# abignoli/EdgeGraph3D

Hardware: AMD Instinct MI355X
Metric: triangulated edge-points/sec (higher is better)
Workload: dtype f64

## Files before the change

edgegraph3d_amd/build.py:

```python
import os
import subprocess
import sys

ROOT = os.path.dirname(os.path.dirname(os.path.abspath(__file__)))
PKG = os.path.join(ROOT, "edgegraph3d_amd")
HOST_DIR = os.path.join(PKG, "host")
CSRC_DIR = os.path.join(PKG, "csrc")
INC_DIR = os.path.join(ROOT, "include")

HOST_LIB = os.path.join(PKG, "libeg3d_host.so")
HIP_LIB = os.path.join(PKG, "libeg3d.so")

HOST_FLAGS = ["-O2", "-std=c++17", "-fPIC", "-shared", "-ffp-contract=off", "-fno-fast-math", "-fopenmp", "-Wall"]
HIP_OPT_FLAGS = ["-O2", "-fno-slp-vectorize", "-fno-vectorize", "-mllvm", "-disable-machine-licm", "-mllvm", "-disable-lsr",
                 "-mllvm", "-enable-pre=false", "-mllvm", "-enable-load-pre=false", "-mllvm", "-enable-misched=false"]
HIP_FLAGS = ["--offload-arch=gfx950"] + HIP_OPT_FLAGS + ["-std=c++17", "-fPIC", "-shared", "-ffp-contract=off",
             "-fno-fast-math", "-fhip-fp32-correctly-rounded-divide-sqrt", "-fno-gpu-rdc",
             "-Wall", "-Wno-unused-function", "-Wno-unused-variable", "-Wno-unused-but-set-variable"]


def _newer(target, sources):
    if not os.path.exists(target):
        return True
    t = os.path.getmtime(target)
# ... 111 lines not shown
    src = os.path.join(PKG, "rccl", "eg3d_rccl.hip")
    deps = [src] + _all_sources(INC_DIR, (".h",)) + _all_sources(os.path.join(PKG, "rccl"), (".h",))
    if force or _newer(RCCL_LIB, deps):
        hipcc = os.environ.get("HIPCC", "/opt/rocm/bin/hipcc")
        _run([hipcc, "--offload-arch=gfx950", "-O2", "-std=c++17", "-fPIC", "-shared", "-I", INC_DIR, src,
              "-L/opt/rocm/lib", "-lrccl", "-Wl,-rpath,/opt/rocm/lib", "-o", RCCL_LIB])
    return RCCL_LIB


RESOURCE_BOUNDS = {
    "k3b_expand_t<4, 0, 0>": {"vgpr_spill_count": 120, "private_segment_fixed_size": 224, "group_segment_fixed_size": 10240},
    "k3b_expand_t<4, 0, 1>": {"vgpr_spill_count": 360, "private_segment_fixed_size": 400, "group_segment_fixed_size": 10240},
    "k3b_expand_t<4, 1, 2>": {"vgpr_spill_count": 140, "private_segment_fixed_size": 256, "group_segment_fixed_size": 10240},
    "k3a_orient": {"vgpr_spill_count": 0, "group_segment_fixed_size": 12800},
    "k3a_follow_spec": {"vgpr_spill_count": 0, "group_segment_fixed_size": 12800},
    "k5_gn_filter": {"vgpr_spill_count": 0},
    "k5_gn_filter<unsigned int, true>": {"vgpr_spill_count": 0, "private_segment_fixed_size": 0, "vgpr_count": 57,
                                         "group_segment_fixed_size": 47124},
    "k5_gn_filter<unsigned long, false>": {"vgpr_spill_count": 0, "private_segment_fixed_size": 0, "group_segment_fixed_size": 48164},
    "k6_compact_scatter": {"vgpr_spill_count": 0, "private_segment_fixed_size": 0, "group_segment_fixed_size": 3104},
    "k7_dedup_claim": {"vgpr_spill_count": 0, "private_segment_fixed_size": 0, "group_segment_fixed_size": 2048},
    "k7_dedup_keep": {"vgpr_spill_count": 0, "private_segment_fixed_size": 0, "group_segment_fixed_size": 16},
    "k8_": {"vgpr_spill_count": 0, "private_segment_fixed_size": 0, "group_segment_fixed_size": 0},
    "k9_": {"vgpr_spill_count": 0, "sgpr_spill_count": 0, "private_segment_fixed_size": 0, "group_segment_fixed_size": 2048},
    "k10_": {"vgpr_spill_count": 0, "sgpr_spill_count": 0, "private_segment_fixed_size": 0, "group_segment_fixed_size": 2048},
    "k11_": {"vgpr_spill_count": 0, "sgpr_spill_count": 0, "private_segment_fixed_size": 0, "group_segment_fixed_size": 32},
    "k12_": {"sgpr_spill_count": 0, "private_segment_fixed_size": 0, "group_segment_fixed_size": 0},
    "k12_keys": {"vgpr_spill_count": 0}, "k12_heads": {"vgpr_spill_count": 0}, "k12_compact": {"vgpr_spill_count": 0},
    "k12_view_off": {"vgpr_spill_count": 0}, "k12_common": {"vgpr_spill_count": 0}, "k12_samples": {"vgpr_spill_count": 0},
    "k12_select": {"vgpr_spill_count": 0}, "k12_final": {"vgpr_spill_count": 0},
# ... 103 lines not shown
```

edgegraph3d_amd/csrc/eg3d_api.hip:

```cpp
#include <hip/hip_runtime.h>
#include <hipcub/hipcub.hpp>

#include <algorithm>
#include <cstdio>
#include <cstdlib>

#include <atomic>
#include <chrono>
#include <cmath>
#include <cstring>
#include <memory>
#include <mutex>
#include <string>
#include <thread>
#include <vector>

#include "../../include/eg3d_host.h"
#include "eg3d_api_internal.h"
#include "eg3d_host_copy.h"

thread_local std::string eg3d::api::g_err;
extern "C" const char* eg3d_last_error(void) { return g_err.c_str(); }

static std::atomic<int64_t> g_live_device_bytes{0};
// ... 931 lines not shown

extern "C" int eg3d_probe_sections_raw(eg3d_ctx* c, double* sum16, uint32_t* n_chains) {
  if (!c || !sum16) return EG3D_ERR_ARG;
  std::vector<ChainOut> co(c->last_nc ? c->last_nc : 1);
  if (c->last_nc) HIP_TRY(hipMemcpy(co.data(), c->b_couts.p, sizeof(ChainOut) * c->last_nc, hipMemcpyDeviceToHost));
  for (int k = 0; k < 16; k++) sum16[k] = 0;
  for (uint32_t j = 0; j < c->last_nc; j++)
    for (int k = 0; k < 16; k++) sum16[k] += (double)co[j].tsec[k];
  if (n_chains) *n_chains = c->last_nc;
  return EG3D_OK;
}

#ifndef EG3D_ONE_SECTION
namespace eg3d { int gn_dbg_read(unsigned long long* out, int reset); }
extern "C" int eg3d_probe_gn(unsigned long long* out128, int reset) { return eg3d::gn_dbg_read(out128, reset); }
#endif

extern "C" int eg3d_probe_hyp_sections(eg3d_ctx* c, double* sum, double* slowest, uint32_t* counts) {
  if (!c || !sum || !slowest || !counts) return EG3D_ERR_ARG;
  const uint32_t n = c->last_nhyp;
  std::vector<HypResult> r(n ? n : 1);
  if (n) HIP_TRY(hipMemcpy(r.data(), c->b_res.p, sizeof(HypResult) * n, hipMemcpyDeviceToHost));
  for (int k = 0; k < 6; k++) sum[k] = slowest[k] = 0;
  for (int k = 0; k < 5; k++) counts[k] = 0;
  counts[0] = n;
  for (uint32_t h = 0; h < n; h++) {
    if (r[h].status & HYP_TRI) counts[1]++;
    if (r[h].status & HYP_D1) counts[2]++;
    if (r[h].status & HYP_D2) counts[3]++;
    if (hyp_compatible(r[h].status, r[h].n1, r[h].n2)) counts[4]++;
// ... 15 lines not shown
```

edgegraph3d_amd/csrc/eg3d_api_internal.h:

```cpp
#pragma once
#include <hip/hip_runtime.h>

#include <algorithm>
#include <chrono>
#include <cstdlib>
#include <cstring>
#include <initializer_list>
#include <memory>
#include <mutex>
#include <string>
#include <vector>

#include "../../include/eg3d.h"
#include "eg3d_kernels.h"
#include "eg3d_k8_replay.h"
#include "eg3d_k9_polymatch.h"
#include "eg3d_k10_simgraph.h"
#include "eg3d_k11_louvain.h"

#define EG3D_API_BEGIN namespace eg3d { namespace api __attribute__((visibility("hidden"))) {
#define EG3D_API_END }}

EG3D_API_BEGIN
extern thread_local std::string g_err;
// ... 175 lines not shown
  WorkBuf prim_tmp;
  WorkBuf k8_cnt, k8_slot, k8_last, k8_firstof, k8_flag, k8_rank, k8_lastof, k8_plid, k8_key[2], k8_val[2], k8_map, k8_sflag, k8_pos;
  WorkBuf g_nodeX, g_nodept, g_pls, g_ple, g_conoff, g_conpl, g_ivoff, g_ivss, g_ivsxy, g_ives, g_ivexy;
  WorkBuf k9_svseed, k9_cnt, k9_pl, k9_dist, k9_acc, k9_accoff, k9_first, k9_parent, k9_root, k9_ckey, k9_rank, k9_key[2], k9_ctr,
      k9_ref, k9_rowoff, k9_plids;
  WorkBuf k10_svseed, k10_cnt, k10_off, k10_pair[2], k10_crkey, k10_cpoff, k10_cpview, k10_cppl, k10_croff, k10_crpoint, k10_weight, k10_vis,
      k10_npairs, k10_pairoff, k10_nkey[2], k10_nodeof, k10_nodeg, k10_nodeview, k10_nodepl, k10_edge[2], k10_dkey[2], k10_dval[2],
      k10_adjoff, k10_adjnode, k10_ctr;
  WorkBuf k11[K11B_COUNT];
  uint32_t louvain_log2_slots = 0;
  uint64_t simgraph_pair_budget = 0;
  int replay_table_bits = 0;
  uint32_t n_pl = 0, n_vtx = 0;
  WorkBuf b_sets_off, b_sets_ids;
  WorkBuf b_fscratch, b_queue, b_items;
  WorkBuf b_pools, b_stage_pts, b_stage_obs, b_stage_used;
  uint32_t slots_per_xcd = 0;
  int k3c_per_cu = 0;
  bool k3b_long_latched = false;
  uint32_t max_pl_vtx = 0;
  uint64_t stage_cap_pts = 0, stage_cap_obs = 0;
  double hits_per_list = 4.0;
  bool hits_learned = false;
  hipEvent_t ea[8], eb[8];
  hipEvent_t ecopy[7] = {nullptr, nullptr, nullptr, nullptr, nullptr, nullptr, nullptr};
  uint32_t chain_cap = 384, pool_cap = 0, hyp_cap = 160;
  uint32_t n_simd = 0;
  int wall_clock_khz = 0;
  double arena_per_hyp = 16.0;
  void* pinned = nullptr;
// ... 112 lines not shown
```

edgegraph3d_amd/csrc/eg3d_api_match.hip:

```cpp
#include <sys/mman.h>

#include <atomic>
#include <condition_variable>
#include <cstdio>
#include <shared_mutex>
#include <thread>

#include "eg3d_api_internal.h"
#include "eg3d_host_copy.h"

#ifndef EG3D_D2H_CHUNK
#define EG3D_D2H_CHUNK ((size_t)16 << 20)
#endif
#define EG3D_D2H_CHUNK_SMALL ((size_t)2 << 20)
#define EG3D_D2H_BIG_CLOUD ((size_t)96 << 20)
#ifndef EG3D_D2H_RING
#define EG3D_D2H_RING 4
#endif
static int ensure_d2h_ring(eg3d_ctx* c, size_t cloud_bytes) {
  const size_t want = cloud_bytes >= EG3D_D2H_BIG_CLOUD ? EG3D_D2H_CHUNK : EG3D_D2H_CHUNK_SMALL;
  if (c->pinned && c->ring_chunk >= want) return EG3D_OK;
  if (c->pinned) (void)hipHostFree(c->pinned);
  c->pinned = nullptr;
  c->ring_chunk = c->pinned_cap = 0;
// ... 303 lines not shown

int follow_and_select(eg3d_ctx* c, BatchState& B, HostOut& H) {
  hipStream_t st = c->stream;
  const uint32_t nt = B.n_tasks;
  BUF_TRY(c->b_res.ensure(sizeof(HypResult) * (B.n_hyp + 1)));
  const uint32_t eng_waves_max = c->n_simd * (uint32_t)(c->tune.k3a_engine_waves > 0 ? c->tune.k3a_engine_waves : 2);
  uint32_t eng_lanes = 64;
  if (c->tune.k3a_engine_lanes > 0)
    eng_lanes = (uint32_t)std::min(64, c->tune.k3a_engine_lanes);
  else
    while (eng_lanes > 8 && (uint64_t)eng_waves_max * (eng_lanes / 2) >= B.n_hyp) eng_lanes /= 2;
  const uint32_t eng_waves = std::max<uint32_t>(1, std::min<uint32_t>(eng_waves_max, (B.n_hyp + eng_lanes - 1) / eng_lanes));
  BUF_TRY(c->b_fscratch.ensure(sizeof(HPoint) * std::min<uint32_t>(c->hyp_cap, EG3D_K3A_STAGE_POINTS) * ((size_t)eng_waves * 64)));
  BUF_TRY(c->b_queue.ensure(4 * sizeof(uint32_t)));
  BUF_TRY(c->b_items.ensure(sizeof(uint32_t) * 2 * ((size_t)B.n_hyp + 1)));
  uint32_t arena_cap = std::max<uint32_t>(1u << 16, std::min<uint64_t>((uint64_t)((double)B.n_hyp * c->arena_per_hyp) + 1, 1ull << 26));
  if (c->tune.arena_cap0) arena_cap = c->tune.arena_cap0;
  Counters hc;
  BUF_TRY(c->b_cs_task.ensure(sizeof(ChainSeed) * (nt + 1)));
  BUF_TRY(c->b_valid.ensure(sizeof(uint32_t) * (nt + 1)));
  BUF_TRY(c->b_chain_off.ensure(sizeof(uint32_t) * (nt + 1)));
  for (int attempt = 0;; attempt++) {
    BUF_TRY(c->b_arena.ensure(sizeof(HPoint) * (size_t)arena_cap));
    HIP_TRY(hipMemsetAsync(c->b_ctr.p, 0, 2 * sizeof(uint32_t), st));
    HIP_TRY(hipEventRecord(c->ea[3], st));
    HIP_TRY(hipMemsetAsync(c->b_queue.p, 0, 4 * sizeof(uint32_t), st));
    launch_k3a_engine(st, eng_waves, eng_waves, eng_lanes, c->ds, B.a, c->b_tasks.as<TaskDesc>(), c->b_hyp_off.as<uint32_t>(),
                      B.n_hyp, c->b_res.as<HypResult>(), c->b_fscratch.as<HPoint>(), c->hyp_cap, c->b_arena.as<HPoint>(),
                      arena_cap, c->b_ctr.as<Counters>(), c->b_queue.as<uint32_t>(), c->b_items.as<uint32_t>());
    HIP_TRY(hipEventRecord(c->eb[3], st));
    HIP_TRY(hipMemsetAsync(c->b_valid.as<uint32_t>() + nt, 0, sizeof(uint32_t), st));
    HIP_TRY(hipEventRecord(c->ea[4], st));
    launch_k3s(st, nt, c->b_hyp_off.as<uint32_t>(), c->b_res.as<HypResult>(), c->b_cs_task.as<ChainSeed>(),
               c->b_valid.as<uint32_t>());
    BUF_TRY(scan_queue_u32(c, c->b_valid.as<uint32_t>(), c->b_chain_off.as<uint32_t>(), nt + 1, 0));
    Readback rb(c);
    const int ic = rb.add(c->b_ctr.p, sizeof(Counters) / 4);
    const int it = rb.add(c->b_chain_off.as<uint32_t>() + nt, 1);
    const int iw = rb.add(c->b_scanchk.as<uint32_t>(), 1);
    rb.clear_after(c->b_scanchk.as<uint32_t>());
    BUF_TRY(rb.run());
    memcpy(&hc, rb.item(ic), sizeof(Counters));
    if (c->tune.trace_arena)
// ... 1003 lines not shown
```

edgegraph3d_amd/csrc/eg3d_k3a_engine.h:

```cpp
#pragma once
#include "eg3d_dev_pipeline.h"

#include "eg3d_dev_coopgn.h"

namespace eg3d {

#ifdef EG3D_GN_COUNTERS
#define K3A_T0() unsigned long long kt_[3] = {0, 0, 0}, kc_[4] = {0, 0, 0, 0}, kt0_ = __builtin_readcyclecounter(), kt1_
#define K3A_T(i) (kt1_ = __builtin_readcyclecounter(), kt_[i] += kt1_ - kt0_, kt0_ = kt1_)
#define K3A_C(i, v) (kc_[i] += (v))
#define K3A_TEND(kern)                                                \
  if (lane == 0) {                                                    \
    for (int q_ = 0; q_ < 3; q_++) EG3D_GN_DBG(113 + 7 * (kern) + q_, kt_[q_]); \
    for (int q_ = 0; q_ < 4; q_++) EG3D_GN_DBG(116 + 7 * (kern) + q_, kc_[q_]); \
  }
#else
#define K3A_T0() ((void)0)
#define K3A_T(i) ((void)0)
#define K3A_C(i, v) ((void)0)
#define K3A_TEND(kern) ((void)0)
#endif

#define EG3D_K3A_STAGE EG3D_K3A_STAGE_POINTS
#ifndef EG3D_K3A_SPEC
#define EG3D_K3A_SPEC 32
#endif

struct K3aShared {
  Obs req[64][3];
  float resX[64][3];
  uint32_t resF[64];
// ... 36 lines not shown
  }
};

__device__ __forceinline__ uint32_t k3a_slots_per_lane(uint32_t n_working) {
  uint32_t k = 64u / n_working, p = 1;
  while (p * 2 <= k && p * 2 <= (uint32_t)EG3D_K3A_SPEC) p *= 2;
  return p;
}

__device__ __forceinline__ void k3a_serve(K3aShared& sh, const DevScene& s, uint32_t lane) {
  __syncthreads();
  if (sh.reqM[lane] & 1u) {
    const Obs o[3] = {sh.req[lane][0], sh.req[lane][1], sh.req[lane][2]};
    float X[3] = {0.0f, 0.0f, 0.0f};
    uint32_t f = 0;
    const bool ok = triangulate3(s.cam_P, o, X, f);
    sh.resX[lane][0] = X[0];
    sh.resX[lane][1] = X[1];
    sh.resX[lane][2] = X[2];
    sh.resF[lane] = (ok ? 1u : 0u) | (f << 8);
  }
  __syncthreads();
}

__device__ __forceinline__ HPoint k3a_point_of_slot(const K3aShared& sh, uint32_t slot) {
  HPoint hp;
  hp.X[0] = sh.resX[slot][0];
  hp.X[1] = sh.resX[slot][1];
  hp.X[2] = sh.resX[slot][2];
  hp.nobs = 3;
  hp.o[0] = sh.req[slot][0];
  hp.o[1] = sh.req[slot][1];
  hp.o[2] = sh.req[slot][2];
  hp.pad = 0;
  return hp;
}

enum : uint32_t { K3A_IDLE = 0, K3A_GEN = 1, K3A_REQ = 2, K3A_END = 3 };
enum : uint32_t { K3A_TRI0 = 0, K3A_ORIENT = 1, K3A_REPLAY = 2, K3A_OPP = 3 };

__global__ void __launch_bounds__(64, EG3D_K3A_WAVES) k3a_orient(DevScene s, StageAView a, const TaskDesc* tasks,
                                                                 const uint32_t* hyp_off, uint32_t n_hyp, HypResult* res,
                                                                 uint32_t cap, HPoint* arena, uint32_t arena_cap,
                                                                 Counters* ctr, uint32_t* queue, uint32_t lanes_per_wave,
                                                                 uint32_t* items, uint32_t* n_items) {
  __shared__ K3aShared sh;
  const uint32_t lane = threadIdx.x;
  const K3aLane L{&sh, lane};
  const unsigned long long lt = (1ull << lane) - 1ull;
  uint32_t st = K3A_IDLE, phase = K3A_TRI0;
  bool exhausted = lane >= lanes_per_wave;
  uint32_t h = 0, t_cur = 0, e = 0, rounds = 0, alive = 0, reqmask = 0, okmask = 0, flags = 0, status = 0;
  uint32_t n1 = 0, n2 = 0, i_rep = 0, base = 0xffffffffu;
  uint32_t dead_round = 0xffffffffu;
  bool arena_ok = false;
  int32_t view[3] = {0, 0, 0};
  uint32_t pl[3] = {0, 0, 0};
  uint32_t dirA = 0, dirB[2] = {0, 0}, dirC[2] = {0, 0};
  uint32_t d1[3] = {0, 0, 0}, d2[3] = {0, 0, 0};
  float X0[3] = {0.0f, 0.0f, 0.0f};
  auto to_hits = [&](const Obs c[3]) {
    PlPt p;
    p.seg = c[0].seg;
    p.x = c[0].x;
    p.y = c[0].y;
// ... 25 lines not shown
    sh.req[slot][0] = o;
    o.view = (uint32_t)view[1];
    o.pl = pl[1];
    o.seg = pB.seg;
    o.x = pB.x;
    o.y = pB.y;
    sh.req[slot][1] = o;
    o.view = (uint32_t)view[2];
    o.pl = pl[2];
    o.seg = pC.seg;
    o.x = pC.x;
    o.y = pC.y;
    sh.req[slot][2] = o;
    sh.reqM[slot] = 1u | ((uint32_t)q << 8) | (round_off << 10);
  };
  K3A_T0();

  for (;;) {
    const unsigned long long working = __ballot(!(st == K3A_IDLE && exhausted));
    if (!working) break;
    K3A_C(0, 1);
    K3A_C(2, __popcll(working));
    const uint32_t K = k3a_slots_per_lane((uint32_t)__popcll(working));
    const uint32_t slot0 = (uint32_t)__popcll(working & lt) * K;
    sh.reqM[lane] = 0;
    __syncthreads();
    uint32_t n_issued = 0;
    if (st == K3A_END) {
      bool finish = false, to_d1 = false, restart = false;
      if (phase == K3A_TRI0) {
        if (okmask & 1u) {
          status |= HYP_TRI;
          e = 0;
          phase = K3A_ORIENT;
          restart = true;
        } else {
          finish = true;
        }
      } else if (phase == K3A_ORIENT) {
        const int amount = __popc(alive);
        if (amount > 1) {
          st = K3A_GEN;
        } else if (amount == 1) {
          to_d1 = true;
        } else if (e == 0) {
          e = 1;
          reload_hits();
          restart = true;
        } else {
          finish = true;
        }
      } else if (phase == K3A_REPLAY) {
        if (i_rep < n1) {
          st = K3A_GEN;
        } else if (e == 0) {
          phase = K3A_OPP;
          dirA = d2[0];
          dirB[0] = d2[1];
          dirC[0] = d2[2];
          alive = 1u;
          reload_hits();
          st = K3A_GEN;
        } else {
          finish = true;
        }
      } else {
        finish = true;
      }
      if (restart) {
        rounds = 0;
        alive = 15u;
        dirA = sh.plr[0][e == 0 ? 2 : 3][lane];
        dirB[0] = sh.plr[1][2][lane];
        dirB[1] = sh.plr[1][3][lane];
        dirC[0] = sh.plr[2][2][lane];
        dirC[1] = sh.plr[2][3][lane];
        st = K3A_GEN;
      }
      if (to_d1) {
        const int qs = __ffs((int)alive) - 1;
        const PlRef pa = L.polyline(s, 0), pb = L.polyline(s, 1), pc = L.polyline(s, 2);
        status |= HYP_D1;
        d1[0] = dirA;
        d1[1] = dirB[qs >> 1];
        d1[2] = dirC[qs & 1];
        d2[0] = (pa.start == d1[0]) ? pa.end : pa.start;
        d2[1] = (pb.start == d1[1]) ? pb.end : pb.start;
        d2[2] = (pc.start == d1[2]) ? pc.end : pc.start;
        if (rounds > cap) flags |= 4u;
        n1 = rounds < cap ? rounds : cap;
        const uint32_t need = n1 + (e == 0 ? 1u : 0u);
        base = atomicAdd(&ctr->arena_used, need);
        arena_ok = base + need <= arena_cap;
        if (!arena_ok) atomicOr(&ctr->flags, CTR_ARENA_OVERFLOW);
        phase = K3A_REPLAY;
        i_rep = 0;
        dirA = d1[0];
        dirB[0] = d1[1];
        dirC[0] = d1[2];
        alive = 1u;
        reload_hits();
        st = K3A_GEN;
      }
      if (finish) {
        HypResult r;
        r.status = status;
        r.n1 = n1;
        r.n2 = n2;
        for (int k = 0; k < 3; k++) {
          r.dirs1[k] = d1[k];
          r.dirs2[k] = d2[k];
          r.X[k] = X0[k];
        }
        r.flags = flags;
        r.pts1_off = ((status & HYP_D1) && arena_ok) ? base : 0xffffffffu;
        r.pts2_off = ((status & HYP_D2) && arena_ok) ? base + n1 : 0xffffffffu;
        res[h] = r;
        if (flags) atomicOr(&ctr->flags, flags);
        if ((status & HYP_D1) && arena_ok) {
          const uint32_t cnt = (status & HYP_D2) ? 2u : 1u;
          const uint32_t at = atomicAdd(n_items, cnt);
          items[at] = 2u * h;
          if (cnt == 2u) items[at + 1] = 2u * h + 1u;
        }
        st = K3A_IDLE;
      }
    }
    if (st == K3A_IDLE && !exhausted) {
      const uint32_t i = atomicAdd(queue, 1u);
      if (i >= n_hyp) {
        exhausted = true;
      } else {
        h = i;
        t_cur = find_owner(hyp_off, a.n_tasks, h);
        const TaskDesc d = tasks[t_cur];
        Obs c[3];
        hypothesis_hits(a, d, t_cur, h - hyp_off[t_cur], c);
        for (int k = 0; k < 3; k++) {
          view[k] = (int32_t)c[k].view;
          pl[k] = c[k].pl;
          L.load_polyline(s, k, view[k], pl[k]);
        }
        to_hits(c);
        status = 0;
        flags = 0;
        n1 = n2 = 0;
        base = 0xffffffffu;
        arena_ok = false;
        for (int k = 0; k < 3; k++) d1[k] = d2[k] = 0;
        X0[0] = X0[1] = X0[2] = 0.0f;
        phase = K3A_TRI0;
        reqmask = 1u;
        okmask = 0;
        st = K3A_REQ;
      }
    }
    dead_round = 0xffffffffu;
    if (st == K3A_GEN) {
      uint32_t walkers = alive;
      for (uint32_t round_off = 0;; round_off++) {
        uint32_t fl = 0, m = walkers;
        const PlRef pa = L.polyline(s, 0);
        PlPt q;
        const uint32_t w = walk_by_distance_pf(pa, L.get(0), dirA, EG3D_FOLLOW_STEP, q);
        if (w & WALK_BAD_DIR) fl |= 8u;
        if (w & WALK_EXTREME) {
          m = 0;
        } else {
          L.set(0, q);
// ... 10 lines not shown
              }
              pk = L.polyline(s, k);
            }
            if (!(m & users)) continue;
            PlPt r;
            const uint32_t wr = walk_by_line_pf(pk, L.get(2 * k - 1 + j), k == 1 ? dirB[j] : dirC[j], la, lb, lc, false, 0.0f,
                                                0.0f, r);
            if (wr & WALK_BAD_DIR) fl |= 8u;
            if (wr & WALK_FOUND)
              L.set(2 * k - 1 + j, r);
            else
              m &= ~users;
          }
        }
        if (phase != K3A_REPLAY) flags |= fl;
        if (round_off == 0) {
          reqmask = m;
          okmask = 0;
          if (!m) {
            if (phase == K3A_REPLAY) n1 = i_rep;
            if (phase == K3A_ORIENT) {
              alive = 0;
              rounds++;
            }
            st = K3A_END;
            break;
          }
          st = K3A_REQ;
          while (reqmask && n_issued < K) {
            const int qq = __ffs((int)reqmask) - 1;
// ... 54 lines not shown
        for (uint32_t j = 0; j < n_issued && !decided; j++) {
          const uint32_t mq = sh.reqM[slot0 + j], f = sh.resF[slot0 + j];
          const uint32_t q = (mq >> 8) & 3u, ro = mq >> 10;
          if (ro != cur) {
            alive = cur == 0 ? okmask : (alive & okmask);
            okmask = 0;
            rounds++;
            cur = ro;
            if (__popc(alive) <= 1) {
              decided = true;
              break;
            }
          }
          if (cur != 0 && !((alive >> q) & 1u)) continue;
          flags |= f >> 8;
          if (f & 1u) okmask |= 1u << q;
        }
        if (decided) {
          st = K3A_END;
        } else if (reqmask) {
          st = K3A_REQ;
        } else {
          alive = cur == 0 ? okmask : (alive & okmask);
          okmask = 0;
          rounds++;
          if (__popc(alive) > 1 && dead_round != 0xffffffffu) {
            alive = 0;
            rounds++;
          }
          st = K3A_END;
        }
      } else {
        const uint32_t f = sh.resF[slot0];
        flags |= f >> 8;
        if (f & 1u) {
          okmask |= 1u;
          if (phase == K3A_TRI0) {
            X0[0] = sh.resX[slot0][0];
            X0[1] = sh.resX[slot0][1];
            X0[2] = sh.resX[slot0][2];
          } else {
            status |= HYP_D2;
            n2 = 1;
            if (arena_ok) arena[base + n1] = k3a_point_of_slot(sh, slot0);
          }
        }
        st = K3A_END;
      }
    }
    K3A_T(2);
  }
  K3A_TEND(0);
}

template <class T>
__device__ __forceinline__ T k3a_pick(const T a[3], int i) {
  return i == 0 ? a[0] : i == 1 ? a[1] : a[2];
}
__device__ __forceinline__ bool k3a_follow_request(const DevScene& s, const K3aLane& L, const int32_t view3[3],
                                                   int st_start, const uint32_t dirs[3], const int32_t ids[3],
// ... 138 lines not shown
        }
        sh.reqM[slot] = 1u | ((uint32_t)st_used << 8) | (fl << 16);
        n_req++;
        for (int k = 0; k < 3; k++) {
          bview[k] = nview[k];
          bpl[k] = npl[k];
          L.set(3 + k, sel_pt[k]);
        }
        st0 = 0;
      }
    }
    K3A_T(0);
    K3A_C(0, 1);
    K3A_C(2, __popcll(working));
    K3A_C(1, __popcll(__ballot(sh.reqM[lane] & 1u)));
    k3a_serve(sh, s, lane);
    K3A_T(1);
    if (have) {
      bool finish = false;
      uint32_t j = 0;
      for (; j < n_req; j++) {
        const uint32_t slot = slot0 + j;
        const uint32_t m = sh.reqM[slot], f = sh.resF[slot];
        flags |= (m >> 16) | (f >> 8);
        if (f & 1u) {
          if (n_init + n_new >= cap) {
            flags |= 4u;
            finish = true;
            break;
          }
// ... 78 lines not shown
```

edgegraph3d_amd/csrc/eg3d_kernels.h:

```cpp
#pragma once
#include <hip/hip_runtime.h>
#include <stdint.h>

#include "eg3d_dev_pipeline.h"

namespace eg3d {

struct SeedsDev {
  const uint32_t* trk_off;
  const int32_t* trk_view;
  const float* trk_xy;
};

__device__ __forceinline__ void seed_obs_in_view(const SeedsDev& sd, uint32_t t0, uint32_t k, int32_t view, float& x,
                                                 float& y) {
  x = 0.f;
  y = 0.f;
  for (uint32_t i = 0; i < k; i++)
    if (sd.trk_view[t0 + i] == view) {
      x = sd.trk_xy[2 * (t0 + i)];
      y = sd.trk_xy[2 * (t0 + i) + 1];
    }
}

// ... 34 lines not shown
               Obs* hits, uint32_t hits_cap, uint32_t stage_cap, Counters* ctr);
struct SetsDev {
  uint32_t n_views;
  const uint32_t* row_off;
  const uint32_t* pl_ids;
};
void launch_n1_samples(hipStream_t st, bool fill, DevScene s, SetsDev sets, uint32_t n_rows, uint32_t item_begin,
                       uint32_t n_items, uint32_t* sample_cnt, const uint32_t* sample_off, Obs* samples,
                       uint32_t* task_seed, uint32_t* task_entry, uint32_t* task_hit, uint32_t* task_list_off,
                       uint32_t* task_row0, Counters* ctr);
void launch_n1_hits(hipStream_t st, bool fill, DevScene s, SetsDev sets, uint32_t n_tasks, const Obs* samples,
                    const uint32_t* task_row0, uint32_t* list_cnt, const uint32_t* list_ptr, Obs* hits, Counters* ctr);
void launch_task_setup(hipStream_t st, StageAView a, const int32_t* map_view, const uint32_t* map_entry,
                       const uint32_t* map_n, TaskDesc* tasks, uint32_t* n_hyp);
#define EG3D_K3A_STAGE_POINTS 16u
void launch_k3a_engine(hipStream_t st, uint32_t orient_waves, uint32_t follow_waves, uint32_t lanes_per_wave, DevScene s,
                       StageAView a, const TaskDesc* tasks, const uint32_t* hyp_off, uint32_t n_hyp, HypResult* res,
                       HPoint* follow_scratch, uint32_t hyp_cap, HPoint* arena, uint32_t arena_cap, Counters* ctr,
                       uint32_t* queue3, uint32_t* items);
void launch_k3s(hipStream_t st, uint32_t n_tasks, const uint32_t* hyp_off, const HypResult* res, ChainSeed* per_task,
                uint32_t* valid);
void launch_compact_chains(hipStream_t st, uint32_t n_tasks, const ChainSeed* per_task, const uint32_t* valid,
                           const uint32_t* chain_off, ChainSeed* chains);
struct SlotPools {
  uint32_t* base;
  uint32_t stride, ring_n, slots_per_xcd;
};
#define EG3D_SMALL_SCENE_VIEWS_HOST 28
#define EG3D_STAGE_VTX_HOST 512
int k3b_blocks_per_cu();
void launch_pool_init(hipStream_t st, SlotPools pools);
#ifdef EG3D_WITH_K3C_ENGINE
int k3c_blocks_per_cu();
void launch_k3c(hipStream_t st, uint32_t n_waves, uint32_t lanes_per_wave, DevScene s, StageAView a, const TaskDesc* tasks,
// ... 84 lines not shown
```

edgegraph3d_amd/csrc/eg3d_kernels.hip:

```cpp
#include <hip/hip_runtime.h>
#include <stdint.h>

#include "eg3d_dev_pipeline.h"
#include "eg3d_dev_coopgn.h"
#include "eg3d_kernels.h"

namespace eg3d {

__device__ __forceinline__ uint32_t wave_min_u32(uint32_t v) {
#pragma unroll
  for (int o = 32; o > 0; o >>= 1) {
    uint32_t t = (uint32_t)__shfl_xor((int)v, o, 64);
    v = t < v ? t : v;
  }
  return v;
}
__device__ __forceinline__ float wave_min_f32(float v) {
#pragma unroll
  for (int o = 32; o > 0; o >>= 1) {
    float t = __shfl_xor(v, o, 64);
    v = t < v ? t : v;
  }
  return v;
}
// ... 1106 lines not shown
                    const uint32_t* task_row0, uint32_t* list_cnt, const uint32_t* list_ptr, Obs* hits, Counters* ctr) {
  if (!n_tasks) return;
  if (fill)
    hipLaunchKernelGGL(k_n1_hits<true>, blocks_for(n_tasks, 256), dim3(256), 0, st, s, sets, n_tasks, samples, task_row0,
                       list_cnt, list_ptr, hits, ctr);
  else
    hipLaunchKernelGGL(k_n1_hits<false>, blocks_for(n_tasks, 256), dim3(256), 0, st, s, sets, n_tasks, samples, task_row0,
                       list_cnt, list_ptr, hits, ctr);
}
void launch_task_setup(hipStream_t st, StageAView a, const int32_t* map_view, const uint32_t* map_entry,
                       const uint32_t* map_n, TaskDesc* tasks, uint32_t* n_hyp) {
  if (!a.n_tasks) return;
  hipLaunchKernelGGL(k_task_setup, blocks_for(a.n_tasks, 256), dim3(256), 0, st, a, map_view, map_entry, map_n, tasks,
                     n_hyp);
}
void launch_k3a_engine(hipStream_t st, uint32_t orient_waves, uint32_t follow_waves, uint32_t lanes_per_wave, DevScene s,
                       StageAView a, const TaskDesc* tasks, const uint32_t* hyp_off, uint32_t n_hyp, HypResult* res,
                       HPoint* follow_scratch, uint32_t hyp_cap, HPoint* arena, uint32_t arena_cap, Counters* ctr,
                       uint32_t* queue3, uint32_t* items) {
  if (!n_hyp) return;
  hipLaunchKernelGGL(k3a_orient, dim3(orient_waves), dim3(64), 0, st, s, a, tasks, hyp_off, n_hyp, res, hyp_cap, arena,
                     arena_cap, ctr, queue3, lanes_per_wave, items, queue3 + 2);
  hipLaunchKernelGGL(k3a_follow_spec, dim3(follow_waves), dim3(64), 0, st, s, res, follow_scratch, hyp_cap, arena, arena_cap, ctr, queue3 + 1, lanes_per_wave, items, queue3 + 2);
}
void launch_k3s(hipStream_t st, uint32_t n_tasks, const uint32_t* hyp_off, const HypResult* res, ChainSeed* per_task,
                uint32_t* valid) {
  if (!n_tasks) return;
  hipLaunchKernelGGL(k3s_select, blocks_for(n_tasks, 256), dim3(256), 0, st, n_tasks, hyp_off, res, per_task, valid);
}
void launch_compact_chains(hipStream_t st, uint32_t n_tasks, const ChainSeed* per_task, const uint32_t* valid,
                           const uint32_t* chain_off, ChainSeed* chains) {
  if (!n_tasks) return;
  hipLaunchKernelGGL(k_compact_chains, blocks_for(n_tasks, 256), dim3(256), 0, st, n_tasks, per_task, valid, chain_off,
                     chains);
}
#ifdef EG3D_GN_COUNTERS
int gn_dbg_read(unsigned long long* out, int reset) {
  if (hipMemcpyFromSymbol(out, HIP_SYMBOL(g_gn_dbg), sizeof(unsigned long long) * 128) != hipSuccess) return -1;
  if (reset) {
    unsigned long long z[128] = {0};
    if (hipMemcpyToSymbol(HIP_SYMBOL(g_gn_dbg), z, sizeof(z)) != hipSuccess) return -1;
  }
  return 0;
}
#endif
static_assert(EG3D_STAGE_VTX_HOST == EG3D_STAGE_VTX, "the host's small-scene rule must match the side walks' staging capacity");
static_assert(EG3D_GN_PACK_MAX >= EG3D_SMALL_SCENE_VIEWS_HOST, "a small scene's solves must fit a packed round");
static_assert(2 * EG3D_SMALL_SCENE_VIEWS_HOST + 8 <= EG3D_COOP_ROWS && 2 * (EG3D_SMALL_SCENE_VIEWS_HOST + 1) + 8 > EG3D_COOP_ROWS,
              "EG3D_SMALL_SCENE_VIEWS_HOST must be the last view count whose N-view step lists fit LDS");
static constexpr auto k3b_expand_small = k3b_expand_t<EG3D_K3B_WAVES, 0, 0>;
static constexpr auto k3b_expand = k3b_expand_t<EG3D_K3B_WAVES, 0, 1>;
#ifndef EG3D_MANY_WAVES
#define EG3D_MANY_WAVES EG3D_K3B_WAVES
#endif
static constexpr auto k3b_expand_many = k3b_expand_t<EG3D_MANY_WAVES, EG3D_MANY_KEEP, 2>;
int k3b_blocks_per_cu() {
// ... 143 lines not shown
```

Baseline: 47.25 million.

## Hoist initial triangulation of all hypotheses into a dense pre-pass kernel

```diff
diff --git a/edgegraph3d_amd/build.py b/edgegraph3d_amd/build.py
--- a/edgegraph3d_amd/build.py
+++ b/edgegraph3d_amd/build.py
@@ -149,6 +149,8 @@
     "k3b_expand_t<4, 1, 2>": {"vgpr_spill_count": 140, "private_segment_fixed_size": 256, "group_segment_fixed_size": 10240},
     "k3a_orient": {"vgpr_spill_count": 0, "group_segment_fixed_size": 12800},
     "k3a_follow_spec": {"vgpr_spill_count": 0, "group_segment_fixed_size": 12800},
+    "k3a_tri0": {"vgpr_spill_count": 0, "sgpr_spill_count": 0, "vgpr_count": 192, "group_segment_fixed_size": 17408},
+    "k3a_pair_count": {"vgpr_spill_count": 0, "private_segment_fixed_size": 0, "group_segment_fixed_size": 0},
     "k5_gn_filter": {"vgpr_spill_count": 0},
     "k5_gn_filter<unsigned int, true>": {"vgpr_spill_count": 0, "private_segment_fixed_size": 0, "vgpr_count": 57,
                                          "group_segment_fixed_size": 47124},
diff --git a/edgegraph3d_amd/csrc/eg3d_api.hip b/edgegraph3d_amd/csrc/eg3d_api.hip
--- a/edgegraph3d_amd/csrc/eg3d_api.hip
+++ b/edgegraph3d_amd/csrc/eg3d_api.hip
@@ -969,6 +969,8 @@
 #ifndef EG3D_ONE_SECTION
 namespace eg3d { int gn_dbg_read(unsigned long long* out, int reset); }
 extern "C" int eg3d_probe_gn(unsigned long long* out128, int reset) { return eg3d::gn_dbg_read(out128, reset); }
+namespace eg3d { int k3a_dbg_read(unsigned long long* out, int reset); }
+extern "C" int eg3d_probe_k3a(unsigned long long* out64, int reset) { return eg3d::k3a_dbg_read(out64, reset); }
 #endif
 
 extern "C" int eg3d_probe_hyp_sections(eg3d_ctx* c, double* sum, double* slowest, uint32_t* counts) {
diff --git a/edgegraph3d_amd/csrc/eg3d_api_internal.h b/edgegraph3d_amd/csrc/eg3d_api_internal.h
--- a/edgegraph3d_amd/csrc/eg3d_api_internal.h
+++ b/edgegraph3d_amd/csrc/eg3d_api_internal.h
@@ -213,6 +213,7 @@
   uint32_t n_pl = 0, n_vtx = 0;
   WorkBuf b_sets_off, b_sets_ids;
   WorkBuf b_fscratch, b_queue, b_items;
+  WorkBuf b_npair, b_pair_off, b_tri0, b_oklist;
   WorkBuf b_pools, b_stage_pts, b_stage_obs, b_stage_used;
   uint32_t slots_per_xcd = 0;
   int k3c_per_cu = 0;
diff --git a/edgegraph3d_amd/csrc/eg3d_api_match.hip b/edgegraph3d_amd/csrc/eg3d_api_match.hip
--- a/edgegraph3d_amd/csrc/eg3d_api_match.hip
+++ b/edgegraph3d_amd/csrc/eg3d_api_match.hip
@@ -341,6 +341,14 @@
   BUF_TRY(c->b_fscratch.ensure(sizeof(HPoint) * std::min<uint32_t>(c->hyp_cap, EG3D_K3A_STAGE_POINTS) * ((size_t)eng_waves * 64)));
   BUF_TRY(c->b_queue.ensure(4 * sizeof(uint32_t)));
   BUF_TRY(c->b_items.ensure(sizeof(uint32_t) * 2 * ((size_t)B.n_hyp + 1)));
+  BUF_TRY(c->b_npair.ensure(sizeof(uint32_t) * (nt + 1)));
+  BUF_TRY(c->b_pair_off.ensure(sizeof(uint32_t) * (nt + 1)));
+  BUF_TRY(c->b_tri0.ensure((size_t)EG3D_K3A_TRI0_BYTES * ((size_t)B.n_hyp + 1)));
+  BUF_TRY(c->b_oklist.ensure(sizeof(uint32_t) * ((size_t)B.n_hyp + 1)));
+  if (B.n_hyp) {
+    launch_k3a_pair_count(st, c->b_tasks.as<TaskDesc>(), nt, c->b_npair.as<uint32_t>());
+    BUF_TRY(scan_queue_u32(c, c->b_npair.as<uint32_t>(), c->b_pair_off.as<uint32_t>(), nt + 1, 0));
+  }
   uint32_t arena_cap = std::max<uint32_t>(1u << 16, std::min<uint64_t>((uint64_t)((double)B.n_hyp * c->arena_per_hyp) + 1, 1ull << 26));
   if (c->tune.arena_cap0) arena_cap = c->tune.arena_cap0;
   Counters hc;
@@ -353,7 +361,8 @@
     HIP_TRY(hipEventRecord(c->ea[3], st));
     HIP_TRY(hipMemsetAsync(c->b_queue.p, 0, 4 * sizeof(uint32_t), st));
     launch_k3a_engine(st, eng_waves, eng_waves, eng_lanes, c->ds, B.a, c->b_tasks.as<TaskDesc>(), c->b_hyp_off.as<uint32_t>(),
-                      B.n_hyp, c->b_res.as<HypResult>(), c->b_fscratch.as<HPoint>(), c->hyp_cap, c->b_arena.as<HPoint>(),
+                      B.n_hyp, c->b_pair_off.as<uint32_t>(), c->b_tri0.p, c->b_oklist.as<uint32_t>(), c->b_res.as<HypResult>(),
+                      c->b_fscratch.as<HPoint>(), c->hyp_cap, c->b_arena.as<HPoint>(),
                       arena_cap, c->b_ctr.as<Counters>(), c->b_queue.as<uint32_t>(), c->b_items.as<uint32_t>());
     HIP_TRY(hipEventRecord(c->eb[3], st));
     HIP_TRY(hipMemsetAsync(c->b_valid.as<uint32_t>() + nt, 0, sizeof(uint32_t), st));
diff --git a/edgegraph3d_amd/csrc/eg3d_k3a_engine.h b/edgegraph3d_amd/csrc/eg3d_k3a_engine.h
--- a/edgegraph3d_amd/csrc/eg3d_k3a_engine.h
+++ b/edgegraph3d_amd/csrc/eg3d_k3a_engine.h
@@ -6,6 +6,8 @@
 namespace eg3d {
 
 #ifdef EG3D_GN_COUNTERS
+__device__ unsigned long long g_k3a_dbg[64];
+#define K3A_DBG(i, v) atomicAdd(&g_k3a_dbg[i], (unsigned long long)(v))
 #define K3A_T0() unsigned long long kt_[3] = {0, 0, 0}, kc_[4] = {0, 0, 0, 0}, kt0_ = __builtin_readcyclecounter(), kt1_
 #define K3A_T(i) (kt1_ = __builtin_readcyclecounter(), kt_[i] += kt1_ - kt0_, kt0_ = kt1_)
 #define K3A_C(i, v) (kc_[i] += (v))
@@ -15,6 +17,7 @@
     for (int q_ = 0; q_ < 4; q_++) EG3D_GN_DBG(116 + 7 * (kern) + q_, kc_[q_]); \
   }
 #else
+#define K3A_DBG(i, v) ((void)0)
 #define K3A_T0() ((void)0)
 #define K3A_T(i) ((void)0)
 #define K3A_C(i, v) ((void)0)
@@ -81,7 +84,22 @@
     const Obs o[3] = {sh.req[lane][0], sh.req[lane][1], sh.req[lane][2]};
     float X[3] = {0.0f, 0.0f, 0.0f};
     uint32_t f = 0;
+#ifdef EG3D_GN_COUNTERS
+    const unsigned long long c0 = __builtin_readcyclecounter();
+    const int mi = (o[1].view < o[0].view) ? (o[2].view < o[1].view ? 2 : 1) : (o[2].view < o[0].view ? 2 : 0);
+    if (o[mi].view == o[2].view) f |= 16u;
+    double Xd[3];
+    dlt2(s.cam_P + (size_t)o[mi].view * 16, o[mi].x, o[mi].y, s.cam_P + (size_t)o[2].view * 16, o[2].x, o[2].y, Xd);
+    const unsigned long long c1 = __builtin_readcyclecounter();
+    const bool ok = gauss_newton3_f64(s.cam_P, o, Xd, X);
+    const unsigned long long c2 = __builtin_readcyclecounter();
+    if (__popcll(__ballot(1) & ((1ull << lane) - 1ull)) == 0) {
+      K3A_DBG(8, c1 - c0);
+      K3A_DBG(9, c2 - c1);
+    }
+#else
     const bool ok = triangulate3(s.cam_P, o, X, f);
+#endif
     sh.resX[lane][0] = X[0];
     sh.resX[lane][1] = X[1];
     sh.resX[lane][2] = X[2];
@@ -103,19 +121,140 @@
   return hp;
 }
 
+struct K3aTri0 {
+  float X[3];
+  uint32_t f;
+};
+#define EG3D_K3A_TRI0_BLOCK 256
+
+__global__ void k3a_pair_count(const TaskDesc* tasks, uint32_t n_tasks, uint32_t* n_pair) {
+  const uint32_t t = blockIdx.x * blockDim.x + threadIdx.x;
+  if (t > n_tasks) return;
+  n_pair[t] = (t < n_tasks && tasks[t].n_hyp) ? tasks[t].cnt[0] * tasks[t].cnt[2] : 0u;
+}
+
+__global__ void __launch_bounds__(EG3D_K3A_TRI0_BLOCK) k3a_tri0(DevScene s, StageAView a, const TaskDesc* tasks,
+                                                               const uint32_t* hyp_off, const uint32_t* pair_off,
+                                                               K3aTri0* tri0, HypResult* res, Counters* ctr,
+                                                               uint32_t* ok_list, uint32_t* n_ok) {
+  __shared__ double X0s[EG3D_K3A_TRI0_BLOCK][3];
+  __shared__ uint32_t p_task[EG3D_K3A_TRI0_BLOCK], p_local[EG3D_K3A_TRI0_BLOCK], cum[EG3D_K3A_TRI0_BLOCK];
+  const uint32_t tid = threadIdx.x;
+  const uint32_t n_pairs = pair_off[a.n_tasks];
+  const uint32_t p0 = blockIdx.x * (uint32_t)EG3D_K3A_TRI0_BLOCK;
+  if (p0 >= n_pairs) return;
+  uint32_t c1n = 0;
+  if (p0 + tid < n_pairs) {
+    const uint32_t t = find_owner(pair_off, a.n_tasks, p0 + tid);
+    const TaskDesc d = tasks[t];
+    const uint32_t local = p0 + tid - pair_off[t];
+    const uint32_t lo = a.task_list_off[t];
+    const Obs h0 = a.hits[a.list_ptr[lo + d.sel_entry[0]] + local / d.cnt[2]];
+    const Obs h2 = a.hits[a.list_ptr[lo + d.sel_entry[2]] + local % d.cnt[2]];
+    double X0[3];
+    dlt2(s.cam_P + (size_t)h0.view * 16, h0.x, h0.y, s.cam_P + (size_t)h2.view * 16, h2.x, h2.y, X0);
+    X0s[tid][0] = X0[0];
+    X0s[tid][1] = X0[1];
+    X0s[tid][2] = X0[2];
+    p_task[tid] = t;
+    p_local[tid] = local;
+    c1n = d.cnt[1];
+    K3A_DBG(1, 1);
+  }
+  cum[tid] = c1n;
+  __syncthreads();
+  for (uint32_t step = 1; step < (uint32_t)EG3D_K3A_TRI0_BLOCK; step <<= 1) {
+    const uint32_t v = tid >= step ? cum[tid - step] : 0u;
+    __syncthreads();
+    cum[tid] += v;
+    __syncthreads();
+  }
+  const uint32_t total = cum[EG3D_K3A_TRI0_BLOCK - 1];
+  for (uint32_t j = tid; j < total; j += (uint32_t)EG3D_K3A_TRI0_BLOCK) {
+    uint32_t q = 0, hi = (uint32_t)EG3D_K3A_TRI0_BLOCK - 1;
+    while (q < hi) {
+      const uint32_t mid = (q + hi) >> 1;
+      if (cum[mid] > j)
+        hi = mid;
+      else
+        q = mid + 1;
+    }
+    const uint32_t i1 = j - (q ? cum[q - 1] : 0u);
+    const uint32_t t = p_task[q], local = p_local[q];
+    const TaskDesc d = tasks[t];
+    const uint32_t lo = a.task_list_off[t];
+    const uint32_t i0 = local / d.cnt[2], i2 = local % d.cnt[2];
+    Obs o[3];
+    o[0] = a.hits[a.list_ptr[lo + d.sel_entry[0]] + i0];
+    o[1] = a.hits[a.list_ptr[lo + d.sel_entry[1]] + i1];
+    o[2] = a.hits[a.list_ptr[lo + d.sel_entry[2]] + i2];
+    const int mi = (o[1].view < o[0].view) ? (o[2].view < o[1].view ? 2 : 1) : (o[2].view < o[0].view ? 2 : 0);
+    uint32_t f = 0;
+    if (o[mi].view == o[2].view) f |= 16u;
+    double X0[3];
+    if (mi == 0) {
+      X0[0] = X0s[q][0];
+      X0[1] = X0s[q][1];
+      X0[2] = X0s[q][2];
+    } else {
+      dlt2(s.cam_P + (size_t)o[mi].view * 16, o[mi].x, o[mi].y, s.cam_P + (size_t)o[2].view * 16, o[2].x, o[2].y, X0);
+    }
+    K3aTri0 z;
+    z.X[0] = z.X[1] = z.X[2] = 0.0f;
+    const bool ok = gauss_newton3_f64(s.cam_P, o, X0, z.X);
+    z.f = (ok ? 1u : 0u) | (f << 8);
+    const uint32_t h = hyp_off[t] + (i0 * d.cnt[1] + i1) * d.cnt[2] + i2;
+    tri0[h] = z;
+    K3A_DBG(0, 1);
+    if (ok) {
+      ok_list[atomicAdd(n_ok, 1u)] = h;
+      K3A_DBG(2, 1);
+    } else {
+      HypResult r;
+      r.status = 0;
+      r.n1 = r.n2 = 0;
+      for (int k = 0; k < 3; k++) {
+        r.dirs1[k] = r.dirs2[k] = 0;
+        r.X[k] = 0.0f;
+      }
+      r.flags = f;
+      r.pts1_off = r.pts2_off = 0xffffffffu;
+      res[h] = r;
+      if (f) atomicOr(&ctr->flags, f);
+    }
+  }
+}
+
 enum : uint32_t { K3A_IDLE = 0, K3A_GEN = 1, K3A_REQ = 2, K3A_END = 3 };
-enum : uint32_t { K3A_TRI0 = 0, K3A_ORIENT = 1, K3A_REPLAY = 2, K3A_OPP = 3 };
+enum : uint32_t { K3A_ORIENT = 1, K3A_REPLAY = 2, K3A_OPP = 3 };
+
+struct K3aKept {
+  float X[3];
+  uint32_t seg[3];
+  float xy[3][2];
+};
+#ifndef EG3D_K3A_KEEP
+#define EG3D_K3A_KEEP 1
+#endif
+static_assert(4 * EG3D_K3A_KEEP * sizeof(K3aKept) <= EG3D_K3A_STAGE_POINTS * sizeof(HPoint), "the kept answers must fit the lane's staging region");
 
 __global__ void __launch_bounds__(64, EG3D_K3A_WAVES) k3a_orient(DevScene s, StageAView a, const TaskDesc* tasks,
-                                                                 const uint32_t* hyp_off, uint32_t n_hyp, HypResult* res,
-                                                                 uint32_t cap, HPoint* arena, uint32_t arena_cap,
-                                                                 Counters* ctr, uint32_t* queue, uint32_t lanes_per_wave,
-                                                                 uint32_t* items, uint32_t* n_items) {
+                                                                 const uint32_t* hyp_off, const K3aTri0* tri0,
+                                                                 const uint32_t* ok_list, const uint32_t* n_ok_p,
+                                                                 HypResult* res, HPoint* scratch, uint32_t cap,
+                                                                 HPoint* arena, uint32_t arena_cap, Counters* ctr,
+                                                                 uint32_t* queue, uint32_t lanes_per_wave, uint32_t* items,
+                                                                 uint32_t* n_items) {
   __shared__ K3aShared sh;
   const uint32_t lane = threadIdx.x;
   const K3aLane L{&sh, lane};
   const unsigned long long lt = (1ull << lane) - 1ull;
-  uint32_t st = K3A_IDLE, phase = K3A_TRI0;
+  const uint32_t n_ok = *n_ok_p;
+  const uint32_t stage = cap < (uint32_t)EG3D_K3A_STAGE ? cap : (uint32_t)EG3D_K3A_STAGE;
+  const uint32_t keep_fit = (uint32_t)((stage * sizeof(HPoint)) / (4 * sizeof(K3aKept)));
+  const uint32_t keep = keep_fit < (uint32_t)EG3D_K3A_KEEP ? keep_fit : (uint32_t)EG3D_K3A_KEEP;
+  K3aKept* const kept = reinterpret_cast<K3aKept*>(scratch + ((size_t)blockIdx.x * 64 + lane) * stage);
+  uint32_t st = K3A_IDLE, phase = K3A_ORIENT;
   bool exhausted = lane >= lanes_per_wave;
   uint32_t h = 0, t_cur = 0, e = 0, rounds = 0, alive = 0, reqmask = 0, okmask = 0, flags = 0, status = 0;
   uint32_t n1 = 0, n2 = 0, i_rep = 0, base = 0xffffffffu;
@@ -171,6 +310,16 @@
     sh.req[slot][2] = o;
     sh.reqM[slot] = 1u | ((uint32_t)q << 8) | (round_off << 10);
   };
+  auto begin_search = [&]() {
+    rounds = 0;
+    alive = 15u;
+    dirA = sh.plr[0][e == 0 ? 2 : 3][lane];
+    dirB[0] = sh.plr[1][2][lane];
+    dirB[1] = sh.plr[1][3][lane];
+    dirC[0] = sh.plr[2][2][lane];
+    dirC[1] = sh.plr[2][3][lane];
+    st = K3A_GEN;
+  };
   K3A_T0();
 
   for (;;) {
@@ -184,17 +333,8 @@
     __syncthreads();
     uint32_t n_issued = 0;
     if (st == K3A_END) {
-      bool finish = false, to_d1 = false, restart = false;
-      if (phase == K3A_TRI0) {
-        if (okmask & 1u) {
-          status |= HYP_TRI;
-          e = 0;
-          phase = K3A_ORIENT;
-          restart = true;
-        } else {
-          finish = true;
-        }
-      } else if (phase == K3A_ORIENT) {
+      bool finish = false, to_d1 = false, to_opp = false;
+      if (phase == K3A_ORIENT) {
         const int amount = __popc(alive);
         if (amount > 1) {
           st = K3A_GEN;
@@ -203,36 +343,17 @@
         } else if (e == 0) {
           e = 1;
           reload_hits();
-          restart = true;
+          begin_search();
         } else {
           finish = true;
         }
       } else if (phase == K3A_REPLAY) {
-        if (i_rep < n1) {
+        if (i_rep < n1)
           st = K3A_GEN;
-        } else if (e == 0) {
-          phase = K3A_OPP;
-          dirA = d2[0];
-          dirB[0] = d2[1];
-          dirC[0] = d2[2];
-          alive = 1u;
-          reload_hits();
-          st = K3A_GEN;
-        } else {
-          finish = true;
-        }
+        else
+          to_opp = true;
       } else {
         finish = true;
-      }
-      if (restart) {
-        rounds = 0;
-        alive = 15u;
-        dirA = sh.plr[0][e == 0 ? 2 : 3][lane];
-        dirB[0] = sh.plr[1][2][lane];
-        dirB[1] = sh.plr[1][3][lane];
-        dirC[0] = sh.plr[2][2][lane];
-        dirC[1] = sh.plr[2][3][lane];
-        st = K3A_GEN;
       }
       if (to_d1) {
         const int qs = __ffs((int)alive) - 1;
@@ -250,14 +371,49 @@
         base = atomicAdd(&ctr->arena_used, need);
         arena_ok = base + need <= arena_cap;
         if (!arena_ok) atomicOr(&ctr->flags, CTR_ARENA_OVERFLOW);
-        phase = K3A_REPLAY;
-        i_rep = 0;
-        dirA = d1[0];
-        dirB[0] = d1[1];
-        dirC[0] = d1[2];
-        alive = 1u;
-        reload_hits();
-        st = K3A_GEN;
+        K3A_DBG(16 + (n1 < 31u ? n1 : 31u), 1);
+        if (n1 <= keep) {
+          K3A_DBG(10, 1);
+          for (uint32_t i = 0; i < n1 && arena_ok; i++) {
+            const K3aKept kp = kept[(uint32_t)qs * keep + i];
+            HPoint hp;
+            hp.nobs = 3;
+            hp.pad = 0;
+            for (int k = 0; k < 3; k++) {
+              hp.X[k] = kp.X[k];
+              hp.o[k].view = (uint32_t)view[k];
+              hp.o[k].pl = pl[k];
+              hp.o[k].seg = kp.seg[k];
+              hp.o[k].x = kp.xy[k][0];
+              hp.o[k].y = kp.xy[k][1];
+            }
+            arena[base + i] = hp;
+          }
+          to_opp = true;
+        } else {
+          K3A_DBG(11, 1);
+          phase = K3A_REPLAY;
+          i_rep = 0;
+          dirA = d1[0];
+          dirB[0] = d1[1];
+          dirC[0] = d1[2];
+          alive = 1u;
+          reload_hits();
+          st = K3A_GEN;
+        }
+      }
+      if (to_opp) {
+        if (e == 0) {
+          phase = K3A_OPP;
+          dirA = d2[0];
+          dirB[0] = d2[1];
+          dirC[0] = d2[2];
+          alive = 1u;
+          reload_hits();
+          st = K3A_GEN;
+        } else {
+          finish = true;
+        }
       }
       if (finish) {
         HypResult r;
@@ -285,10 +441,11 @@
     }
     if (st == K3A_IDLE && !exhausted) {
       const uint32_t i = atomicAdd(queue, 1u);
-      if (i >= n_hyp) {
+      if (i >= n_ok) {
         exhausted = true;
       } else {
-        h = i;
+        h = ok_list[i];
+        const K3aTri0 z = tri0[h];
         t_cur = find_owner(hyp_off, a.n_tasks, h);
         const TaskDesc d = tasks[t_cur];
         Obs c[3];
@@ -299,17 +456,19 @@
           L.load_polyline(s, k, view[k], pl[k]);
         }
         to_hits(c);
-        status = 0;
-        flags = 0;
+        status = HYP_TRI;
+        flags = z.f >> 8;
         n1 = n2 = 0;
         base = 0xffffffffu;
         arena_ok = false;
         for (int k = 0; k < 3; k++) d1[k] = d2[k] = 0;
-        X0[0] = X0[1] = X0[2] = 0.0f;
-        phase = K3A_TRI0;
-        reqmask = 1u;
-        okmask = 0;
-        st = K3A_REQ;
+        X0[0] = z.X[0];
+        X0[1] = z.X[1];
+        X0[2] = z.X[2];
+        phase = K3A_ORIENT;
+        e = 0;
+        reqmask = okmask = 0;
+        begin_search();
       }
     }
     dead_round = 0xffffffffu;
@@ -350,6 +509,14 @@
           }
         }
         if (phase != K3A_REPLAY) flags |= fl;
+#ifdef EG3D_GN_COUNTERS
+        if (m && phase == K3A_ORIENT) {
+          K3A_DBG(3, __popc(m));
+          K3A_DBG(4, __popc(m) - ((m & 5u) ? 1 : 0) - ((m & 10u) ? 1 : 0));
+        } else if (m) {
+          K3A_DBG(phase == K3A_REPLAY ? 5 : 6, 1);
+        }
+#endif
         if (round_off == 0) {
           reqmask = m;
           okmask = 0;
@@ -434,7 +601,20 @@
           }
           if (cur != 0 && !((alive >> q) & 1u)) continue;
           flags |= f >> 8;
-          if (f & 1u) okmask |= 1u << q;
+          if (f & 1u) {
+            okmask |= 1u << q;
+            if (rounds < keep) {
+              const uint32_t slot = slot0 + j;
+              K3aKept kp;
+              for (int k = 0; k < 3; k++) {
+                kp.X[k] = sh.resX[slot][k];
+                kp.seg[k] = sh.req[slot][k].seg;
+                kp.xy[k][0] = sh.req[slot][k].x;
+                kp.xy[k][1] = sh.req[slot][k].y;
+              }
+              kept[q * keep + rounds] = kp;
+            }
+          }
         }
         if (decided) {
           st = K3A_END;
@@ -455,15 +635,9 @@
         flags |= f >> 8;
         if (f & 1u) {
           okmask |= 1u;
-          if (phase == K3A_TRI0) {
-            X0[0] = sh.resX[slot0][0];
-            X0[1] = sh.resX[slot0][1];
-            X0[2] = sh.resX[slot0][2];
-          } else {
-            status |= HYP_D2;
-            n2 = 1;
-            if (arena_ok) arena[base + n1] = k3a_point_of_slot(sh, slot0);
-          }
+          status |= HYP_D2;
+          n2 = 1;
+          if (arena_ok) arena[base + n1] = k3a_point_of_slot(sh, slot0);
         }
         st = K3A_END;
       }
@@ -632,6 +806,7 @@
     K3A_C(0, 1);
     K3A_C(2, __popcll(working));
     K3A_C(1, __popcll(__ballot(sh.reqM[lane] & 1u)));
+    K3A_DBG(7, n_req);
     k3a_serve(sh, s, lane);
     K3A_T(1);
     if (have) {
diff --git a/edgegraph3d_amd/csrc/eg3d_kernels.h b/edgegraph3d_amd/csrc/eg3d_kernels.h
--- a/edgegraph3d_amd/csrc/eg3d_kernels.h
+++ b/edgegraph3d_amd/csrc/eg3d_kernels.h
@@ -72,10 +72,12 @@
 void launch_task_setup(hipStream_t st, StageAView a, const int32_t* map_view, const uint32_t* map_entry,
                        const uint32_t* map_n, TaskDesc* tasks, uint32_t* n_hyp);
 #define EG3D_K3A_STAGE_POINTS 16u
+#define EG3D_K3A_TRI0_BYTES 16u
+void launch_k3a_pair_count(hipStream_t st, const TaskDesc* tasks, uint32_t n_tasks, uint32_t* n_pair);
 void launch_k3a_engine(hipStream_t st, uint32_t orient_waves, uint32_t follow_waves, uint32_t lanes_per_wave, DevScene s,
-                       StageAView a, const TaskDesc* tasks, const uint32_t* hyp_off, uint32_t n_hyp, HypResult* res,
-                       HPoint* follow_scratch, uint32_t hyp_cap, HPoint* arena, uint32_t arena_cap, Counters* ctr,
-                       uint32_t* queue3, uint32_t* items);
+                       StageAView a, const TaskDesc* tasks, const uint32_t* hyp_off, uint32_t n_hyp, const uint32_t* pair_off,
+                       void* tri0, uint32_t* ok_list, HypResult* res, HPoint* follow_scratch, uint32_t hyp_cap, HPoint* arena,
+                       uint32_t arena_cap, Counters* ctr, uint32_t* queue4, uint32_t* items);
 void launch_k3s(hipStream_t st, uint32_t n_tasks, const uint32_t* hyp_off, const HypResult* res, ChainSeed* per_task,
                 uint32_t* valid);
 void launch_compact_chains(hipStream_t st, uint32_t n_tasks, const ChainSeed* per_task, const uint32_t* valid,
diff --git a/edgegraph3d_amd/csrc/eg3d_kernels.hip b/edgegraph3d_amd/csrc/eg3d_kernels.hip
--- a/edgegraph3d_amd/csrc/eg3d_kernels.hip
+++ b/edgegraph3d_amd/csrc/eg3d_kernels.hip
@@ -1144,14 +1144,21 @@
   hipLaunchKernelGGL(k_task_setup, blocks_for(a.n_tasks, 256), dim3(256), 0, st, a, map_view, map_entry, map_n, tasks,
                      n_hyp);
 }
+static_assert(sizeof(K3aTri0) == EG3D_K3A_TRI0_BYTES, "the host sizes the TRI0 records by EG3D_K3A_TRI0_BYTES");
+void launch_k3a_pair_count(hipStream_t st, const TaskDesc* tasks, uint32_t n_tasks, uint32_t* n_pair) {
+  hipLaunchKernelGGL(k3a_pair_count, blocks_for(n_tasks + 1, 256), dim3(256), 0, st, tasks, n_tasks, n_pair);
+}
 void launch_k3a_engine(hipStream_t st, uint32_t orient_waves, uint32_t follow_waves, uint32_t lanes_per_wave, DevScene s,
-                       StageAView a, const TaskDesc* tasks, const uint32_t* hyp_off, uint32_t n_hyp, HypResult* res,
-                       HPoint* follow_scratch, uint32_t hyp_cap, HPoint* arena, uint32_t arena_cap, Counters* ctr,
-                       uint32_t* queue3, uint32_t* items) {
+                       StageAView a, const TaskDesc* tasks, const uint32_t* hyp_off, uint32_t n_hyp, const uint32_t* pair_off,
+                       void* tri0, uint32_t* ok_list, HypResult* res, HPoint* follow_scratch, uint32_t hyp_cap, HPoint* arena,
+                       uint32_t arena_cap, Counters* ctr, uint32_t* queue4, uint32_t* items) {
   if (!n_hyp) return;
-  hipLaunchKernelGGL(k3a_orient, dim3(orient_waves), dim3(64), 0, st, s, a, tasks, hyp_off, n_hyp, res, hyp_cap, arena,
-                     arena_cap, ctr, queue3, lanes_per_wave, items, queue3 + 2);
-  hipLaunchKernelGGL(k3a_follow_spec, dim3(follow_waves), dim3(64), 0, st, s, res, follow_scratch, hyp_cap, arena, arena_cap, ctr, queue3 + 1, lanes_per_wave, items, queue3 + 2);
+  hipLaunchKernelGGL(k3a_tri0, blocks_for(n_hyp, EG3D_K3A_TRI0_BLOCK), dim3(EG3D_K3A_TRI0_BLOCK), 0, st, s, a, tasks, hyp_off,
+                     pair_off, static_cast<K3aTri0*>(tri0), res, ctr, ok_list, queue4 + 3);
+  hipLaunchKernelGGL(k3a_orient, dim3(orient_waves), dim3(64), 0, st, s, a, tasks, hyp_off, static_cast<const K3aTri0*>(tri0),
+                     ok_list, queue4 + 3, res, follow_scratch, hyp_cap, arena, arena_cap, ctr, queue4, lanes_per_wave, items,
+                     queue4 + 2);
+  hipLaunchKernelGGL(k3a_follow_spec, dim3(follow_waves), dim3(64), 0, st, s, res, follow_scratch, hyp_cap, arena, arena_cap, ctr, queue4 + 1, lanes_per_wave, items, queue4 + 2);
 }
 void launch_k3s(hipStream_t st, uint32_t n_tasks, const uint32_t* hyp_off, const HypResult* res, ChainSeed* per_task,
                 uint32_t* valid) {
@@ -1170,6 +1177,14 @@
   if (reset) {
     unsigned long long z[128] = {0};
     if (hipMemcpyToSymbol(HIP_SYMBOL(g_gn_dbg), z, sizeof(z)) != hipSuccess) return -1;
+  }
+  return 0;
+}
+int k3a_dbg_read(unsigned long long* out, int reset) {
+  if (hipMemcpyFromSymbol(out, HIP_SYMBOL(g_k3a_dbg), sizeof(unsigned long long) * 64) != hipSuccess) return -1;
+  if (reset) {
+    unsigned long long z[64] = {0};
+    if (hipMemcpyToSymbol(HIP_SYMBOL(g_k3a_dbg), z, sizeof(z)) != hipSuccess) return -1;
   }
   return 0;
 }
```

Result: no change. 47.44 million, median of 6 (+0.4%).
